# jinlong17/DA-Detect

Measured on AMD Instinct MI355X. Metric: train images/sec, DA-Faster-RCNN R-50 Cityscapes->Foggy, higher is better.
Workload: dtype f32

## Files before the change

da_detect_amd/_C.py:

```python
import contextlib
import os
import ctypes
import time

import torch

from . import _lib
from . import amax as _amax
from . import weights as _weights
from ._lib import ConvDesc

CL = torch.channels_last

NMS_TIE_RULE = 0

PROFILER = None
_KNAME_CACHE = {}


class KernelProfiler(object):

    def __init__(self, pool=0, only=None):
        self.only = only
        self._pool = []
# ... 686 lines not shown
def maxpool3x3s2_relu_backward(y, gp, scale=None):
    _dev(y, "y"), _dev(gp, "gp")
    y, gp = _nhwc(y), _nhwc(gp)
    N, C, H, W = y.shape
    Ho, Wo = (H + 2 - 3) // 2 + 1, (W + 2 - 3) // 2 + 1
    assert tuple(gp.shape) == (N, C, Ho, Wo), "maxpool3x3s2_relu_backward: gp %s for y %s" % (tuple(gp.shape), tuple(y.shape))
    g = torch.empty((N, C, H, W), dtype=torch.float32, device=y.device, memory_format=CL)
    slot = _amax.new_slot(y.device) if _mode4() else None
    _lib.call("dadet_maxpool3x3s2_relu_backward", _p(y), _p(gp), _p(scale), _p(g), N, H, W, C, Ho, Wo,
              ctypes.c_void_p(slot[0]) if slot else None, _stream())
    if slot:
        _amax.attach(g, slot)
    return g


def avgpool_forward(x):
    _dev(x, "x")
    x = _nhwc(x)
    R, C, h, w = x.shape
    y = torch.empty((R, C), dtype=torch.float32, device=x.device)
    _lib.call("dadet_avgpool_forward", _p(x), _p(y), R, h * w, C, _stream())
    return _amax.carry(y, x)


def avgpool_backward(gy, h, w):
    _dev(gy, "gy")
    gy = gy.contiguous()
    R, C = gy.shape
    gx = torch.empty((R, C, h, w), dtype=torch.float32, device=gy.device, memory_format=CL)
    _lib.call("dadet_avgpool_backward", _p(gy), _p(gx), R, h * w, C, _stream())
    return _amax.carry(gx, gy)


def nchw3_to_nhwc4(x):
    _dev(x, "x")
    x = x.contiguous()
    N, C, H, W = x.shape
    assert C == 3
    y = torch.empty((N, 4, H, W), dtype=torch.float32, device=x.device, memory_format=CL)
    _lib.call("dadet_nchw3_to_nhwc4", _p(x), _p(y), N, H, W, _stream())
    if _mode4():
        _amax.ptr(x)
        _amax.carry(y, x)
    return y


def two_image_ends(r_cst, n_src):
    return min(max(int(n_src), 0), int(r_cst)), int(r_cst)


def da_ins_tail_forward(h, w3, b3, labels, means, r_bce, r_cst, n_src):
    return da_ins_tail_forward_n(h, w3, b3, labels, means, r_bce, r_cst, two_image_ends(r_cst, n_src))


def da_ins_tail_backward(h, w3, logits, labels, means, coef, inv_keep, r_bce, r_cst, n_src):
    return da_ins_tail_backward_n(h, w3, logits, labels, means, coef, inv_keep, r_bce, r_cst, two_image_ends(r_cst, n_src))


def _row_ends(row_end):
    ends = [int(e) for e in row_end]
    return (ctypes.c_int * len(ends))(*ends), len(ends)


def da_ins_tail_forward_n(h, w3, b3, labels, means, r_bce, r_cst, row_end):
    _dev(h, "h")
    rows, C = h.shape
# ... 655 lines not shown
```

da_detect_amd/_lib.py:

```python
import ctypes
import os
from ctypes import POINTER, c_char_p, c_float, c_int, c_int64, c_size_t, c_uint64, c_void_p

_HERE = os.path.dirname(os.path.abspath(__file__))
LIB_PATH = os.environ.get("DADET_LIB") or os.path.join(_HERE, "libdadet_hip.so")
_lib = None
DEFAULT_GEMM_MODE = "4"


class ConvDesc(ctypes.Structure):

    _fields_ = [(n, c_int) for n in (
        "N", "H", "W", "Cin", "Cout", "KH", "KW", "stride", "pad", "Ho", "Wo", "OutH", "OutW",
        "out_spatial_stride", "relu_mode")]


class ConvPlanInfo(ctypes.Structure):

    _fields_ = [(n, c_int) for n in (
        "family", "variant", "tiles_m", "tiles_n", "ksplit", "splits", "rows_per_split", "sk_dp_tiles", "sk_tiles", "sk_units",
        "sk_iters", "sk_max_parts", "big_splits", "big_body", "launches", "grid", "needs_counters")] + [
        ("workspace_bytes", c_size_t), ("name", ctypes.c_char * 64)]


# ... 126 lines not shown
    "dadet_gather_pixel_taps_level": [_P, _P, _P, c_int, c_int, c_int, c_int, c_int, c_int, c_int, c_int, c_int, _P, _P],
    "dadet_scatter_pixel_taps_add_level": [_P, _P, _P, c_int, c_int, c_int, c_int, c_int, c_int, c_int, c_int, c_int, _P,
                                           _P],
    "dadet_gather_pixel_taps": [_P, _P, c_int, c_int, c_int, c_int, c_int, c_int, c_int, c_int, _P, _P],
    "dadet_scatter_pixel_taps_add": [_P, _P, c_int, c_int, c_int, c_int, c_int, c_int, c_int, c_int, _P, _P],
    "dadet_fast_rcnn_loss": [_P, _P, c_int, c_int, _P, _P, c_int, _P, _P, _P, c_int, _P, _P, _P, _P],
    "dadet_fast_rcnn_loss_rows": [_P, _P, c_int, c_int, c_int, _P, _P, _P, _P, _P, _P],
    "dadet_sample_rois": [_P, _P, _P, c_int, c_int, c_int, c_uint64, c_int, _P, _P, _P, _P, _P, _P, _P, _P],
    "dadet_proposals_sample": [_P, _P, _P, _P, c_int, _P, c_int, _P, _P, c_int, c_float, c_float, c_float, c_float, c_float,
                               c_float, c_int, c_int, c_uint64, c_int, _P, _P, _P, _P, _P, _P, _P, _P, _P, _P, _P, _P],
    "dadet_sample_anchors": [_P, _P, c_int, c_int, c_int, c_uint64, c_int64, _P, _P, _P, _P, _P],
    "dadet_topk_sorted": [_P, c_int, c_int, c_int64, c_int, _P, _P, _P],
    "dadet_topk_sorted_rows_workspace_bytes": [c_int, c_int, POINTER(c_size_t)],
    "dadet_topk_sorted_rows": [POINTER(TopkRow), c_int, _P, c_size_t, _P],
    "dadet_rpn_anchor_targets": [_P, _P, c_int, _P, c_int, c_float, c_float, _P, _P, _P, _P],
    "dadet_box_match_encode": [_P, c_int, _P, _P, c_int, c_float, c_float, c_float, c_float, c_float, c_float, _P, _P,
                               _P, _P],
    "dadet_roi_pool_forward": [_P, _P, _P, _P, c_int, c_int, c_int, c_int, c_int, c_int, c_int, c_float, _P],
    "dadet_roi_pool_backward": [_P, _P, _P, _P, c_int, c_int, c_int, c_int, c_int, c_int, c_int, _P],
    "dadet_deform_psroi_pool_forward": [_P, _P, _P, _P, _P, c_int, c_int, c_int, c_int, c_int, c_int, c_float,
                                        c_int, c_int, c_int, c_int, c_int, c_float, c_int, _P],
    "dadet_deform_psroi_pool_backward": [_P, _P, _P, _P, _P, _P, _P, c_int, c_int, c_int, c_int, c_int, c_int,
                                         c_float, c_int, c_int, c_int, c_int, c_int, c_float, c_int, _P],
    "dadet_relu_bn_backward": [_P, _P, _P, _P, _P, c_int64, c_int, _P],
    "dadet_relu_bn_backward_m": [_P, _P, _P, _P, _P, c_int64, c_int, _P, _P, _P],
    "dadet_colsum_workspace_bytes": [c_int64, c_int, POINTER(c_size_t)],
    "dadet_colsum": [_P, _P, c_int64, c_int, _P, c_size_t, _P],
    "dadet_colsum_ld": [_P, c_int, _P, c_int64, c_int, c_int, _P, c_size_t, _P],
    "dadet_channel_affine": [_P, _P, _P, _P, c_int64, c_int, c_int, _P],
    "dadet_maxpool3x3s2_forward": [_P, _P, c_int, c_int, c_int, c_int, c_int, c_int, _P],
    "dadet_maxpool3x3s2_relu_backward": [_P, _P, _P, _P, c_int, c_int, c_int, c_int, c_int, c_int, _P, _P],
    "dadet_avgpool_forward": [_P, _P, c_int, c_int, c_int, _P],
    "dadet_avgpool_backward": [_P, _P, c_int, c_int, c_int, _P],
    "dadet_nchw3_to_nhwc4": [_P, _P, c_int, c_int, c_int, _P],
    "dadet_rpn_decode_clip": [_P, _P, _P, c_int, c_float, c_float, c_float, c_float, c_float, c_float, c_float, _P, _P],
    "dadet_da_img_head_loss_forward": [_P, _P, _P, _P, _P, _P, c_int, c_int, c_int, _P],
    "dadet_da_img_head_loss_backward": [_P, _P, _P, _P, _P, _P, _P, _P, _P, c_int, c_int, c_int, _P],
    "dadet_da_img_head_loss_backward_g": [_P, _P, _P, _P, _P, _P, _P, c_float, c_float, _P, _P, _P, _P, c_int, c_int, c_int,
                                          _P],
    "dadet_da_img_head_loss_backward_gm": [_P, _P, _P, _P, _P, _P, _P, c_float, c_float, _P, _P, _P, _P, c_int, c_int, c_int,
                                          _P, _P, _P],
    "dadet_da_ins_tail_forward": [_P, _P, _P, _P, _P, _P, _P, c_int, c_int, c_int, c_int, c_int, _P],
    "dadet_da_ins_tail_backward": [_P, _P, _P, _P, _P, _P, c_float, _P, _P, _P, _P, c_int, c_int, c_int, c_int, c_int, _P],
    "dadet_da_ins_tail_forward_n": [_P, _P, _P, _P, _P, _P, _P, c_int, c_int, POINTER(c_int), c_int, c_int, c_int, _P],
    "dadet_da_ins_tail_backward_n": [_P, _P, _P, _P, _P, _P, c_float, _P, _P, _P, _P, c_int, c_int, POINTER(c_int), c_int,
                                     c_int, c_int, _P],
    "dadet_da_ins_dropout_rows": [_P, _P, _P, c_int64, c_int, _P],
    "dadet_da_ins_merge": [_P, _P, _P, _P, _P, _P, c_int64, c_int, _P],
    "dadet_triplet_w_forward": [_P, _P, _P, c_int, c_int, c_int, c_float, c_float, _P, _P, _P],
    "dadet_triplet_w_backward": [_P, _P, _P, _P, _P, c_int, c_int, c_int, c_float, c_float, _P, _P, _P, _P],
    "dadet_sgd_step": [_P, c_int, c_int64, c_float, c_int, c_float, _P],
}
_RESTYPES = {"dadet_last_error": c_char_p}
EXPORTED_SYMBOLS = sorted(list(_SIGNATURES) + ["dadet_last_error"])


class DadetError(RuntimeError):
    pass


def load():
    global _lib
    if _lib is not None:
        return _lib
    if not os.path.exists(LIB_PATH):
        raise DadetError(
# ... 27 lines not shown
```

da_detect_amd/csrc/elementwise.hip:

```cpp
#include "box_match.h"
#include "conv_common.h"
#include <float.h>

namespace dadet {

static inline int stream_blocks(int64_t work_items, int threads) {
  int64_t b = ceil_div64(work_items, threads);
  if (b > kMaxStreamBlocks) b = kMaxStreamBlocks;
  if (b < 1) b = 1;
  return (int)b;
}

__global__ void relu_bn_backward_kernel(const float4* __restrict__ g, const float4* __restrict__ y,
                                        const float4* __restrict__ scale, float4* __restrict__ g_out,
                                        float4* __restrict__ g_scaled, int64_t total4, int C4,
                                        unsigned* __restrict__ amax_out, unsigned* __restrict__ amax_scaled) {
  float mo = 0.f, ms = 0.f;
  for (int64_t i = (int64_t)blockIdx.x * blockDim.x + threadIdx.x; i < total4;
       i += (int64_t)gridDim.x * blockDim.x) {
    const float4 gv = g[i];
    float4 r = gv;
    if (y) {
      const float4 yv = y[i];
      r.x = yv.x > 0.f ? gv.x : 0.f;
// ... 158 lines not shown
}

__global__ void avgpool_fwd_kernel(const float4* __restrict__ x, float4* __restrict__ y, int R, int HW,
                                   int C4) {
  const int64_t total = (int64_t)R * C4;
  const float inv = (float)HW;
  for (int64_t i = (int64_t)blockIdx.x * blockDim.x + threadIdx.x; i < total;
       i += (int64_t)gridDim.x * blockDim.x) {
    const int c = (int)(i % C4);
    const int64_t r = i / C4;
    float4 a = make_float4(0.f, 0.f, 0.f, 0.f);
    for (int p = 0; p < HW; ++p) {
      const float4 v = x[(r * HW + p) * C4 + c];
      a.x += v.x; a.y += v.y; a.z += v.z; a.w += v.w;
    }
    a.x /= inv; a.y /= inv; a.z /= inv; a.w /= inv;
    y[i] = a;
  }
}
__global__ void avgpool_bwd_kernel(const float4* __restrict__ gy, float4* __restrict__ gx, int R, int HW,
                                   int C4) {
  const int64_t total = (int64_t)R * HW * C4;
  const float inv = (float)HW;
  for (int64_t i = (int64_t)blockIdx.x * blockDim.x + threadIdx.x; i < total;
       i += (int64_t)gridDim.x * blockDim.x) {
    const int c = (int)(i % C4);
    const int64_t r = i / ((int64_t)HW * C4);
    float4 g = gy[r * C4 + c];
    g.x /= inv; g.y /= inv; g.z /= inv; g.w /= inv;
    gx[i] = g;
  }
}

__global__ void nchw3_to_nhwc4_kernel(const float* __restrict__ x, float4* __restrict__ y, int N,
                                      int64_t HW) {
  const int64_t total = (int64_t)N * HW;
  for (int64_t i = (int64_t)blockIdx.x * blockDim.x + threadIdx.x; i < total;
       i += (int64_t)gridDim.x * blockDim.x) {
    const int64_t n = i / HW, p = i % HW;
    const float* b = x + n * 3 * HW + p;
    y[i] = make_float4(b[0], b[HW], b[2 * HW], 0.f);
  }
}

__global__ void rpn_decode_clip_kernel(const float4* __restrict__ deltas, const float4* __restrict__ anchors,
                                       const int64_t* __restrict__ topk_idx, int K, float wx, float wy,
                                       float ww, float wh, float xform_clip, float im_w, float im_h,
                                       float4* __restrict__ out) {
  const int k = blockIdx.x * blockDim.x + threadIdx.x;
  if (k >= K) return;
  const int64_t a = topk_idx[k];
  const float4 b = anchors[a];
  const float4 d = deltas[a];
  const float width = b.z - b.x + 1.f;
  const float height = b.w - b.y + 1.f;
  const float ctr_x = b.x + 0.5f * width;
  const float ctr_y = b.y + 0.5f * height;
  const float dx = d.x / wx, dy = d.y / wy;
  float dw = d.z / ww, dh = d.w / wh;
  dw = fminf(dw, xform_clip);
  dh = fminf(dh, xform_clip);
  const float pcx = dx * width + ctr_x;
  const float pcy = dy * height + ctr_y;
  const float pw = expf(dw) * width;
  const float ph = expf(dh) * height;
  float x1 = pcx - 0.5f * pw;
// ... 302 lines not shown
  DADET_REQUIRE(N >= 0 && H > 0 && W > 0 && C > 0 && C % 4 == 0, "maxpool_relu_backward: bad dims");
  DADET_REQUIRE(Ho == (H + 2 - 3) / 2 + 1 && Wo == (W + 2 - 3) / 2 + 1, "maxpool_relu_backward: Ho/Wo mismatch");
  if (N == 0) return DADET_OK;
  DADET_REQUIRE(y && gp && g && aligned16(y) && aligned16(gp) && aligned16(scale) && aligned16(g),
                "maxpool_relu_backward: bad pointers");
  DADET_REQUIRE((int64_t)N * H * W < (1LL << 31), "maxpool_relu_backward: tensor too large for 32-bit pixel indexing");
  const int64_t total = (int64_t)N * H * W * (C / 4);
  hipLaunchKernelGGL(maxpool3x3s2_relu_backward_kernel, dim3(stream_blocks(total, 256)), dim3(256), 0, as_stream(stream),
                     reinterpret_cast<const float4*>(y), reinterpret_cast<const float4*>(gp),
                     reinterpret_cast<const float4*>(scale), reinterpret_cast<float4*>(g), N, H, W, C / 4, Ho, Wo,
                     reinterpret_cast<unsigned*>(amax_out));
  return check_launch("maxpool3x3s2_relu_backward");
}

extern "C" int dadet_avgpool_forward(const float* x, float* y, int R, int HW, int C, void* stream) {
  DADET_REQUIRE(R >= 0 && HW > 0 && C > 0 && C % 4 == 0, "avgpool: bad dims");
  if (R == 0) return DADET_OK;
  DADET_REQUIRE(x && y && aligned16(x) && aligned16(y), "avgpool: bad pointers");
  hipLaunchKernelGGL(avgpool_fwd_kernel, dim3(stream_blocks((int64_t)R * (C / 4), 256)), dim3(256), 0,
                     as_stream(stream), reinterpret_cast<const float4*>(x), reinterpret_cast<float4*>(y), R,
                     HW, C / 4);
  return check_launch("avgpool_forward");
}
extern "C" int dadet_avgpool_backward(const float* gy, float* gx, int R, int HW, int C, void* stream) {
  DADET_REQUIRE(R >= 0 && HW > 0 && C > 0 && C % 4 == 0, "avgpool_backward: bad dims");
  if (R == 0) return DADET_OK;
  DADET_REQUIRE(gy && gx && aligned16(gy) && aligned16(gx), "avgpool_backward: bad pointers");
  hipLaunchKernelGGL(avgpool_bwd_kernel, dim3(stream_blocks((int64_t)R * HW * (C / 4), 256)), dim3(256), 0,
                     as_stream(stream), reinterpret_cast<const float4*>(gy), reinterpret_cast<float4*>(gx),
                     R, HW, C / 4);
  return check_launch("avgpool_backward");
}

extern "C" int dadet_nchw3_to_nhwc4(const float* x, float* y, int N, int H, int W, void* stream) {
  DADET_REQUIRE(N >= 0 && H > 0 && W > 0, "nchw3_to_nhwc4: bad dims");
  if (N == 0) return DADET_OK;
  DADET_REQUIRE(x && y && aligned16(y), "nchw3_to_nhwc4: bad pointers");
  const int64_t HW = (int64_t)H * W;
  hipLaunchKernelGGL(nchw3_to_nhwc4_kernel, dim3(stream_blocks((int64_t)N * HW, 256)), dim3(256), 0,
                     as_stream(stream), x, reinterpret_cast<float4*>(y), N, HW);
  return check_launch("nchw3_to_nhwc4");
}

extern "C" int dadet_rpn_decode_clip(const float* deltas, const float* anchors, const int64_t* topk_idx,
                                     int K, float wx, float wy, float ww, float wh, float xform_clip,
                                     float im_w, float im_h, float* boxes_out, void* stream) {
  DADET_REQUIRE(K >= 0, "rpn_decode_clip: K < 0");
  if (K == 0) return DADET_OK;
  DADET_REQUIRE(deltas && anchors && topk_idx && boxes_out, "rpn_decode_clip: null pointer");
  DADET_REQUIRE(aligned16(deltas) && aligned16(anchors) && aligned16(boxes_out),
                "rpn_decode_clip: pointers must be 16-byte aligned");
  hipLaunchKernelGGL(rpn_decode_clip_kernel, dim3(ceil_div(K, 256)), dim3(256), 0, as_stream(stream),
                     reinterpret_cast<const float4*>(deltas), reinterpret_cast<const float4*>(anchors),
                     topk_idx, K, wx, wy, ww, wh, xform_clip, im_w, im_h,
                     reinterpret_cast<float4*>(boxes_out));
  return check_launch("rpn_decode_clip");
}

extern "C" int dadet_rpn_anchor_targets(const float* anchors, const unsigned char* visible, int A,
                                        const float* gt_boxes, int G, float high_threshold, float low_threshold,
                                        unsigned* workspace_G, float* labels, float* regression_targets,
                                        void* stream) {
  DADET_REQUIRE(A >= 0 && G > 0, "rpn_anchor_targets: needs A >= 0 anchors and G > 0 ground-truth boxes");
  if (A == 0) return DADET_OK;
  DADET_REQUIRE(anchors && visible && gt_boxes && workspace_G && labels && regression_targets,
                "rpn_anchor_targets: null pointer");
// ... 71 lines not shown
```

da_detect_amd/layers/misc.py:

```python

import torch
from torch import nn
from torch.autograd import Function
from torch.autograd.function import once_differentiable

from .. import _C
from .. import amax as _amax
from .conv import conv2d_affine_act

CL = torch.channels_last


class FrozenBatchNorm2d(nn.Module):

    def __init__(self, n):
        super(FrozenBatchNorm2d, self).__init__()
        self.register_buffer("weight", torch.ones(n))
        self.register_buffer("bias", torch.zeros(n))
        self.register_buffer("running_mean", torch.zeros(n))
        self.register_buffer("running_var", torch.ones(n))
        self._cache = None

    def folded(self):
        key = (self.weight._version, self.bias._version, self.running_mean._version,
               self.running_var._version, self.weight.device)
        if self._cache is None or self._cache[0] != key:
            scale = self.weight * self.running_var.rsqrt()
            shift = self.bias - self.running_mean * scale
            self._cache = (key, scale.contiguous(), shift.contiguous())
        return self._cache[1], self._cache[2]

    def forward(self, x):
        scale, shift = self.folded()
        return _ChannelAffine.apply(x, scale, shift)


class _ChannelAffine(Function):
    @staticmethod
    def forward(ctx, x, scale, shift):
# ... 235 lines not shown
    @staticmethod
    def forward(ctx, logits, targets, gamma, alpha):
        ctx.save_for_backward(logits, targets)
        ctx.num_classes, ctx.gamma, ctx.alpha = logits.shape[1], gamma, alpha
        return _C.sigmoid_focalloss_forward(logits, targets, ctx.num_classes, gamma, alpha)

    @staticmethod
    @once_differentiable
    def backward(ctx, d_loss):
        logits, targets = ctx.saved_tensors
        return _C.sigmoid_focalloss_backward(logits, targets, d_loss.contiguous(), ctx.num_classes, ctx.gamma,
                                             ctx.alpha), None, None, None


sigmoid_focal_loss = _SigmoidFocalLoss.apply


class SigmoidFocalLoss(nn.Module):

    def __init__(self, gamma, alpha):
        super(SigmoidFocalLoss, self).__init__()
        self.gamma, self.alpha = gamma, alpha

    def forward(self, logits, targets):
        return sigmoid_focal_loss(logits, targets, self.gamma, self.alpha).sum()

    def __repr__(self):
        return "{}(gamma={}, alpha={})".format(self.__class__.__name__, self.gamma, self.alpha)


class _AvgPoolHW(Function):

    @staticmethod
    def forward(ctx, x):
        ctx.hw = (x.shape[2], x.shape[3])
        return _C.avgpool_forward(x)

    @staticmethod
    @once_differentiable
    def backward(ctx, g):
        return _C.avgpool_backward(g, *ctx.hw)


_POOL_MEMO = True


def global_avg_pool(x):
    if x.shape[0] == 0:
        return x.new_empty((0, x.shape[1]))
    memo = x.__dict__.get("_dadet_pooled") if _POOL_MEMO else None
    if memo is not None and memo[0] == x._version and memo[1] == torch.is_grad_enabled():
        return memo[2]
    y = _AvgPoolHW.apply(x)
    x._dadet_pooled = (x._version, torch.is_grad_enabled(), y)
    return y
```

da_detect_amd/modeling/backbone/resnet.py:

```python
import weakref
from collections import namedtuple

import torch
import torch.nn.functional as F
from torch import nn

from ... import _C
from ...layers import Conv2d, FrozenBatchNorm2d, conv2d_affine_act
from ...utils.registry import Registry
from ...utils import streams
from ...utils.streams import WgradLane
from ...weights import Stamp

StageSpec = namedtuple("StageSpec", ["index", "block_count", "return_features"])


def _specs(*rows):
    return tuple(StageSpec(index=i, block_count=c, return_features=r) for (i, c, r) in rows)


ResNet50StagesTo5 = _specs((1, 3, False), (2, 4, False), (3, 6, False), (4, 3, True))
ResNet50StagesTo4 = _specs((1, 3, False), (2, 4, False), (3, 6, True))
ResNet101StagesTo5 = _specs((1, 3, False), (2, 4, False), (3, 23, False), (4, 3, True))
ResNet101StagesTo4 = _specs((1, 3, False), (2, 4, False), (3, 23, True))
ResNet50FPNStagesTo5 = _specs((1, 3, True), (2, 4, True), (3, 6, True), (4, 3, True))
ResNet101FPNStagesTo5 = _specs((1, 3, True), (2, 4, True), (3, 23, True), (4, 3, True))
ResNet152FPNStagesTo5 = _specs((1, 3, True), (2, 8, True), (3, 36, True), (4, 3, True))


_WGRAD_BATCH = True
_WGRAD_GROUP = __import__("os").environ.get("DADET_WGRAD_GROUP", "1") == "1"


class _WgradGroup(object):

    _known = {}

    def __init__(self, lane, batch, weights):
        self.lane, self.batch, self.reqs = lane, batch, []
        self.on = (_WGRAD_GROUP and batch is not None and _C._mode4() and 2 <= len(weights) <= _C.WGRAD_GROUP_MAX
# ... 6 lines not shown
    def take(self, w, xin, gout, stride, pad, scale, shape=None):
        if not self.on:
            return False
        self.reqs.append(dict(x=xin, gy=gout, weight_shape=tuple(w.shape) if shape is None else shape, stride=stride,
                              pad=pad, out_scale=scale, dw=streams.direct_grad_target(w), accumulate=True))
        return True

    def issue(self):
        if not self.reqs:
            return
        reqs, batch = self.reqs, self.batch
        key = self.key + tuple((tuple(r["x"].shape), r["stride"]) for r in reqs)

        def run():
            ok = self._known.get(key, True) and _C.conv_wgrad_group(reqs, batch)
            if not ok:
                self._known[key] = self._known[self.key] = False
                for r in reqs:
                    _C.conv_wgrad(r["x"], r["gy"], r["weight_shape"], r["stride"], r["pad"], out_scale=r["out_scale"],
                                  dw=r["dw"], accumulate=True, pending=batch)

        self.lane.run_group(run, *[t for r in reqs for t in (r["x"], r["gy"])])
        self.reqs = []


class _BlockBackward(object):

    def __init__(self, needs, x, w1, wd, s1, sd, stride):
        self.need_x, self.n1, self.n2, self.n3, nd = needs
        self.nd = nd and wd is not None
        self.x, self.w1, self.wd, self.s1, self.sd, self.stride = x, w1, wd, s1, sd, stride

    def open(self, G, out, out_private, y2, w2, w3, s3):
        self.S3 = G.contiguous(memory_format=torch.channels_last) if out_private else _C.relu_bn_backward(G, out, None)[1]
        self.lane = WgradLane(G.device, rows=G.shape[0] * G.shape[2] * G.shape[3])
        self.batch = _C.WgradBatch() if _WGRAD_BATCH else None
        weights = ((w3, self.n3), (w2, self.n2), (self.w1, self.n1), (self.wd, self.nd))
        self.group = _WgradGroup(self.lane, self.batch, [w for w, need in weights if need])
        dw3 = self.wgrad(w3, y2, self.S3, 1, 0, s3) if self.n3 else None
        return _C.conv_forward(self.S3, _C.conv_weight_transpose(w3, s3), relu_mode=2, mask_ref=y2), dw3

    def wgrad(self, w, xin, gout, st, pd, sc, shape=None, grouped=True):
        shape = tuple(w.shape) if shape is None else shape
        batch = self.batch
        if grouped and self.group.take(w, xin, gout, st, pd, sc, shape=shape):
            return None
        return self.lane.run_into(w, lambda acc: _C.conv_wgrad(xin, gout, shape, st, pd, out_scale=sc, dw=acc,
                                                               accumulate=True, pending=batch),
                                  lambda: _C.conv_wgrad(xin, gout, shape, st, pd, out_scale=sc, pending=batch),
                                  xin, gout)

    def close(self, S1, in_relu):
        x, w1, wd, s1, sd, stride, S3 = self.x, self.w1, self.wd, self.s1, self.sd, self.stride, self.S3
        dw1 = dwd = dx = None
        if self.n1:
            dw1 = self.wgrad(w1, x, S1, stride, 0, s1)
        if self.nd:
            dwd = self.wgrad(wd, x, S3, stride, 0, sd)
        self.group.issue()
        self.lane.reduce_batch(self.batch)
        if self.need_x:
            gate = dict(relu_mode=2, mask_ref=x) if in_relu else {}
            hw = tuple(x.shape[2:])
            if wd is None:
                dx = _C.conv_forward(S1, _C.conv_weight_transpose(w1, s1), addend=S3, **gate)
            elif stride == 1:
                t = _C.conv_forward(S3, _C.conv_weight_transpose(wd, sd))
# ... 148 lines not shown
        self.downsample = None
        if in_channels != out_channels:
            self.downsample = nn.Sequential(
                Conv2d(in_channels, out_channels, kernel_size=1, stride=stride, bias=False),
                norm_func(out_channels))
            nn.init.kaiming_uniform_(self.downsample[0].weight, a=1)
        stride_1x1, stride_3x3 = (stride, 1) if stride_in_1x1 else (1, stride)
        self.conv1 = Conv2d(in_channels, bottleneck_channels, kernel_size=1, stride=stride_1x1, bias=False)
        self.bn1 = norm_func(bottleneck_channels)
        self.with_dcn = bool(dcn_config.get("stage_with_dcn", False))
        if self.with_dcn:
            from ...layers.dcn import DFConv2d
            self.conv2 = DFConv2d(bottleneck_channels, bottleneck_channels,
                                  with_modulated_dcn=dcn_config.get("with_modulated_dcn", False), kernel_size=3,
                                  stride=stride_3x3, groups=num_groups, dilation=dilation,
                                  deformable_groups=dcn_config.get("deformable_groups", 1), bias=False)
        else:
            self.conv2 = Conv2d(bottleneck_channels, bottleneck_channels, kernel_size=3, stride=stride_3x3,
                                padding=1, bias=False)
        self.bn2 = norm_func(bottleneck_channels)
        self.conv3 = Conv2d(bottleneck_channels, out_channels, kernel_size=1, bias=False)
        self.bn3 = norm_func(out_channels)
        for l in (self.conv1, self.conv3) + (() if self.with_dcn else (self.conv2,)):
            nn.init.kaiming_uniform_(l.weight, a=1)

    def forward(self, x, in_relu=False, out_private=False, stride=None):
        if self.with_dcn:
            assert stride is None
            if self._dcn_fusable(x):
                c2 = self.conv2
                wd = sd = bd = None
                if self.downsample is not None:
                    wd, (sd, bd) = self.downsample[0].weight, self.downsample[1].folded()
                return _DCNBottleneckFn.apply(x, self.conv1.weight, c2.conv.weight, self.conv3.weight, wd,
                                              c2.offset.weight, c2.offset.bias, *self.bn1.folded(), *self.bn2.folded(),
                                              *self.bn3.folded(), sd, bd, self.conv1.stride[0], in_relu, out_private,
                                              c2.with_modulated_dcn, c2.conv.deformable_groups)
            return self._forward_dcn(x)
        if self.conv2.stride[0] == 1:
            if x.shape[0] == 0 and stride is None:
                return self._forward_per_conv(x)
            wd = sd = bd = None
            if self.downsample is not None:
                wd, (sd, bd) = self.downsample[0].weight, self.downsample[1].folded()
            return _BottleneckFn.apply(x, self.conv1.weight, self.conv2.weight, self.conv3.weight, wd,
                                       *self.bn1.folded(), *self.bn2.folded(), *self.bn3.folded(), sd, bd,
                                       self.conv1.stride[0] if stride is None else stride, in_relu, out_private)
        assert stride is None
        return self._forward_per_conv(x)

    def input_is_strided_1x1(self):
        s = self.conv1.stride[0]
        if (self.uses_fused_path() and s > 1 and self.downsample is not None and self.conv1.kernel_size == (1, 1)
                and self.downsample[0].kernel_size == (1, 1) and self.downsample[0].stride[0] == s):
            return s
        return 1

    def uses_fused_path(self):
        if self.with_dcn:
            return self._dcn_fusable(None)
        return self.conv2.stride[0] == 1

    def _dcn_fusable(self, x):
        c = self.conv2.conv
        ok = (_DCN_FUSED and c.stride == 1 and c.dilation == 1 and c.groups == 1 and c.bias is None
              and c.kernel_size == (3, 3) and c.in_channels % (4 * c.deformable_groups) == 0)
        return ok and (x is None or (x.is_cuda and x.shape[0] > 0))

    def _forward_dcn(self, x):
        out = self.conv1(x, *self.bn1.folded(), relu=True)
        out = F.relu(self.bn2(self.conv2(out)))
        identity = x if self.downsample is None else self.downsample[0](x, *self.downsample[1].folded())
        return self.conv3(out, *self.bn3.folded(), residual=identity, relu=True)

    def _forward_per_conv(self, x):
        out = self.conv1(x, *self.bn1.folded(), relu=True)
        out = self.conv2(out, *self.bn2.folded(), relu=True)
        identity = x if self.downsample is None else self.downsample[0](x, *self.downsample[1].folded())
        return self.conv3(out, *self.bn3.folded(), residual=identity, relu=True)

# ... 180 lines not shown
```

da_detect_amd/modeling/rpn/rpn.py:

```python
import os

import torch
from torch import nn

from ...layers import Conv2d, conv1x1_multi
from ...layers.misc import rpn_head_loss_rows, rpn_head_loss_rows_pyramid
from .. import registry
from ..box_coder import BoxCoder
from .anchor_generator import make_anchor_generator
from .inference import make_rpn_postprocessor
from .loss import make_rpn_loss_evaluator
from ..elision import elision_enabled, leading_source_images
from ...utils.streams import record, side_section, side_stream



@registry.RPN_HEADS.register("SingleConvRPNHead")
class RPNHead(nn.Module):

    def __init__(self, cfg, in_channels, num_anchors):
        super(RPNHead, self).__init__()
        self.conv = Conv2d(in_channels, in_channels, kernel_size=3, stride=1, padding=1)
        self.cls_logits = Conv2d(in_channels, num_anchors, kernel_size=1, stride=1)
        self.bbox_pred = Conv2d(in_channels, num_anchors * 4, kernel_size=1, stride=1)
        for l in (self.conv, self.cls_logits, self.bbox_pred):
            torch.nn.init.normal_(l.weight, std=0.01)
            torch.nn.init.constant_(l.bias, 0)

    keep_hidden = False

    def forward(self, x):
        logits, bbox_reg = [], []
        self.hidden = []
        for feature in x:
            t = self.conv(feature, relu=True)
            if self.keep_hidden:
                self.hidden.append(t)
            cls, box = conv1x1_multi(t, [self.cls_logits.weight, self.bbox_pred.weight],
                                     [self.cls_logits.bias, self.bbox_pred.bias])
            logits.append(cls)
            bbox_reg.append(box)
        return logits, bbox_reg


_ROW_BACKWARD = __import__("os").environ.get("DADET_RPN_ROW_BACKWARD", "1") == "1"


class _InjectGrad(torch.autograd.Function):

    @staticmethod
    def forward(ctx, x, g, e, event):
        ctx.event = event
        ctx.save_for_backward(*[t for t in (g, e) if t is not None])
        ctx.has = (g is not None, e is not None)
        from ... import amax
        return amax.carry(x.view_as(x), x)

    @staticmethod
    def backward(ctx, grad_out):
        saved = list(ctx.saved_tensors)
        g = saved.pop(0) if ctx.has[0] else None
        e = saved.pop(0) if ctx.has[1] else None
        if ctx.event is not None:
            torch.cuda.current_stream(grad_out.device).wait_event(ctx.event)
        out = grad_out + e if e is not None else None
        if g is not None:
            if out is None and g.shape[0] == grad_out.shape[0]:
                out = grad_out + g
            else:
                out = grad_out.clone() if out is None else out
                out[:g.shape[0]] += g
        return out, None, None, None


class RPNModule(torch.nn.Module):

    early_backward = False
    live_images = None
    after_early_backward = None

    def __init__(self, cfg):
        super(RPNModule, self).__init__()
        self.cfg = cfg.clone()
        anchor_generator = make_anchor_generator(cfg)
        in_channels = cfg.MODEL.BACKBONE.OUT_CHANNELS
        head = registry.RPN_HEADS[cfg.MODEL.RPN.RPN_HEAD](cfg, in_channels,
                                                         anchor_generator.num_anchors_per_location()[0])
        rpn_box_coder = BoxCoder(weights=(1.0, 1.0, 1.0, 1.0))
        self.anchor_generator = anchor_generator
        self.head = head
        self.box_selector_train = make_rpn_postprocessor(cfg, rpn_box_coder, is_train=True)
        self.box_selector_test = make_rpn_postprocessor(cfg, rpn_box_coder, is_train=False)
        self.loss_evaluator = make_rpn_loss_evaluator(cfg, rpn_box_coder)
        self.proposals_ready = None
        self._feature_grads = None
        self.inputs_ready = None

# ... 143 lines not shown
```

include/dadet.h:

```cpp
#ifndef DADET_H_
#define DADET_H_

#include <stddef.h>
#include <stdint.h>

#ifdef __cplusplus
extern "C" {
#endif

#define DADET_OK 0
#define DADET_EINVAL (-1)
#define DADET_ELAUNCH (-2)
#define DADET_EWORKSPACE (-3)
#define DADET_EUNSUPPORTED (-4)

const char* dadet_last_error(void);
int dadet_version(void);
int dadet_device_info(int* cu_count, int* clock_khz, size_t* hbm_bytes, char* arch_name, int arch_name_len);

int dadet_nms_workspace_bytes(int n, size_t* bytes_out);
int dadet_nms(const float* boxes_xyxy, const float* scores, int n, float thresh, int tie_rule,
              int max_keep, void* workspace, size_t workspace_bytes, int64_t* keep_out,
              int* num_keep_out, void* stream);
int dadet_nms_batch_workspace_bytes(int batch, int n_max, size_t* bytes_out);
// ... 296 lines not shown

int dadet_box_match_encode(const float* proposals, int P, const float* gt_boxes, const int64_t* gt_labels, int G,
                           float high_threshold, float low_threshold, float wx, float wy, float ww, float wh,
                           int64_t* matched_idxs, int64_t* labels, float* regression_targets, void* stream);

int dadet_deform_psroi_pool_forward(const float* data, const float* rois, const float* trans, float* out,
                                    float* top_count, int B, int H, int W, int C, int R, int no_trans,
                                    float spatial_scale, int output_dim, int group_size, int pooled_size,
                                    int part_size, int sample_per_part, float trans_std, int num_classes,
                                    void* stream);
int dadet_deform_psroi_pool_backward(const float* grad_out, const float* top_count, const float* data,
                                     const float* rois, const float* trans, float* grad_data, float* grad_trans,
                                     int B, int H, int W, int C, int R, int no_trans, float spatial_scale,
                                     int output_dim, int group_size, int pooled_size, int part_size,
                                     int sample_per_part, float trans_std, int num_classes, void* stream);

int dadet_relu_bn_backward(const float* g, const float* y, const float* scale, float* g_out,
                           float* g_scaled, int64_t rows, int C, void* stream);
int dadet_relu_bn_backward_m(const float* g, const float* y, const float* scale, float* g_out, float* g_scaled,
                             int64_t rows, int C, float* amax_out, float* amax_scaled, void* stream);
int dadet_colsum_workspace_bytes(int64_t rows, int C, size_t* bytes_out);
int dadet_colsum_ld(const float* g, int ld, float* out, int64_t rows, int C, int accumulate, void* workspace,
                    size_t workspace_bytes, void* stream);
int dadet_colsum(const float* g, float* out, int64_t rows, int C, void* workspace, size_t workspace_bytes,
                 void* stream);
int dadet_channel_affine(const float* x, const float* scale, const float* bias, float* y, int64_t rows,
                         int C, int relu, void* stream);
int dadet_maxpool3x3s2_forward(const float* x, float* y, int N, int H, int W, int C, int Ho, int Wo,
                               void* stream);
int dadet_maxpool3x3s2_relu_backward(const float* y, const float* gp, const float* scale, float* g, int N, int H,
                                     int W, int C, int Ho, int Wo, float* amax_out, void* stream);
int dadet_avgpool_forward(const float* x, float* y, int R, int HW, int C, void* stream);
int dadet_avgpool_backward(const float* gy, float* gx, int R, int HW, int C, void* stream);
int dadet_nchw3_to_nhwc4(const float* x, float* y, int N, int H, int W, void* stream);

int dadet_rpn_decode_clip(const float* deltas, const float* anchors, const int64_t* topk_idx, int K,
                          float wx, float wy, float ww, float wh, float xform_clip, float im_w,
                          float im_h, float* boxes_out, void* stream);

int dadet_da_img_head_loss_forward(const float* t, const float* w2, const float* b2, const float* labels,
                                   float* logits_out, float* sums_out, int num_images,
                                   int rows_per_image, int C1, void* stream);
int dadet_da_img_head_loss_backward(const float* t, const float* w2, const float* logits,
                                    const float* labels, const float* coef, float* g_t_w, float* g_t_x,
                                    float* g_w2, float* g_b2, int num_images, int rows_per_image, int C1,
                                    void* stream);
int dadet_da_img_head_loss_backward_g(const float* t, const float* w2, const float* logits, const float* labels,
                                      const float* g_bce, const float* g_mean_sig, const float* w_adv_dev, float w_adv,
                                      float w_cst, float* g_t_w, float* g_t_x, float* g_w2, float* g_b2, int num_images,
                                      int rows_per_image, int C1, void* stream);
int dadet_da_img_head_loss_backward_gm(const float* t, const float* w2, const float* logits, const float* labels,
                                       const float* g_bce, const float* g_mean_sig, const float* w_adv_dev, float w_adv,
                                       float w_cst, float* g_t_w, float* g_t_x, float* g_w2, float* g_b2, int num_images,
                                       int rows_per_image, int C1, float* amax_w, float* amax_x, void* stream);
int dadet_da_ins_tail_forward(const float* h, const float* w3, const float* b3, const float* labels,
                              const float* means, float* logits, float* sums, int R_bce, int R_cst, int n_src,
                              int levels, int C, void* stream);
int dadet_da_ins_tail_backward(const float* h, const float* w3, const float* logits, const float* labels,
                               const float* means, const float* coef, float inv_keep, float* g_z, float* g_w3,
                               float* g_b3, float* g_means, int R_bce, int R_cst, int n_src, int levels, int C,
                               void* stream);
int dadet_da_ins_tail_forward_n(const float* h, const float* w3, const float* b3, const float* labels,
                                const float* means, float* logits, float* sums, int R_bce, int R_cst,
                                const int* row_end, int num_images, int levels, int C, void* stream);
int dadet_da_ins_tail_backward_n(const float* h, const float* w3, const float* logits, const float* labels,
                                 const float* means, const float* coef, float inv_keep, float* g_z, float* g_w3,
// ... 26 lines not shown
```

Before: 170.8.

## Fuse ReLU gating into gradient junction and lazy avgpool backward

Adds two fused kernels. One sums the incoming gradient with the side-branch gradients and applies the ReLU mask of the backbone output in a single pass. The other expands the avgpool gradient and applies the ReLU mask directly. Tensors are tagged so the bottleneck backward can skip its own relu_bn_backward pass when the gradient is already gated, or materialise the pooled gradient lazily. This removes full-size elementwise passes and intermediate tensors over large feature maps, at the cost of version-tagged metadata that must stay correct across autograd.

```diff
diff --git a/da_detect_amd/_C.py b/da_detect_amd/_C.py
--- a/da_detect_amd/_C.py
+++ b/da_detect_amd/_C.py
@@ -742,6 +742,39 @@
     return _amax.carry(gx, gy)
 
 
+def avgpool_backward_gated(gy, y):
+    _dev(gy, "gy"), _dev(y, "y")
+    gy = gy.contiguous()
+    y = _nhwc(y)
+    R, C, h, w = y.shape
+    assert tuple(gy.shape) == (R, C)
+    gx = torch.empty((R, C, h, w), dtype=torch.float32, device=gy.device, memory_format=CL)
+    slot = _amax.new_slot(gy.device) if _mode4() and R > 0 else None
+    _lib.call("dadet_avgpool_backward_gated", _p(gy), _p(y), _p(gx), ctypes.c_void_p(slot[0]) if slot else None, R, h * w, C,
+              _stream())
+    if slot:
+        _amax.attach(gx, slot)
+    return gx
+
+
+def grad_junction(grad, y, e=None, g=None):
+    _dev(grad, "grad"), _dev(y, "y")
+    grad, y = _nhwc(grad), _nhwc(y)
+    assert grad.shape == y.shape
+    B, C, H, W = y.shape
+    e = _nhwc(e) if e is not None else None
+    g = _nhwc(g) if g is not None else None
+    assert e is None or e.shape == y.shape
+    assert g is None or (tuple(g.shape[1:]) == (C, H, W) and g.shape[0] <= B)
+    out = torch.empty_like(grad)
+    slot = _amax.new_slot(y.device) if _mode4() and grad.numel() > 0 else None
+    _lib.call("dadet_grad_junction", _p(grad), _p(e), _p(g), 0 if g is None else g.shape[0] * H * W, _p(y), _p(out),
+              ctypes.c_void_p(slot[0]) if slot else None, B * H * W, C, _stream())
+    if slot:
+        _amax.attach(out, slot)
+    return out
+
+
 def nchw3_to_nhwc4(x):
     _dev(x, "x")
     x = x.contiguous()
diff --git a/da_detect_amd/_lib.py b/da_detect_amd/_lib.py
--- a/da_detect_amd/_lib.py
+++ b/da_detect_amd/_lib.py
@@ -182,6 +182,8 @@
     "dadet_maxpool3x3s2_relu_backward": [_P, _P, _P, _P, c_int, c_int, c_int, c_int, c_int, c_int, _P, _P],
     "dadet_avgpool_forward": [_P, _P, c_int, c_int, c_int, _P],
     "dadet_avgpool_backward": [_P, _P, c_int, c_int, c_int, _P],
+    "dadet_avgpool_backward_gated": [_P, _P, _P, _P, c_int, c_int, c_int, _P],
+    "dadet_grad_junction": [_P, _P, _P, c_int64, _P, _P, _P, c_int64, c_int, _P],
     "dadet_nchw3_to_nhwc4": [_P, _P, c_int, c_int, c_int, _P],
     "dadet_rpn_decode_clip": [_P, _P, _P, c_int, c_float, c_float, c_float, c_float, c_float, c_float, c_float, _P, _P],
     "dadet_da_img_head_loss_forward": [_P, _P, _P, _P, _P, _P, c_int, c_int, c_int, _P],
diff --git a/da_detect_amd/csrc/elementwise.hip b/da_detect_amd/csrc/elementwise.hip
--- a/da_detect_amd/csrc/elementwise.hip
+++ b/da_detect_amd/csrc/elementwise.hip
@@ -214,6 +214,51 @@
   }
 }
 
+__global__ void avgpool_bwd_gated_kernel(const float4* __restrict__ gy, const float4* __restrict__ y,
+                                         float4* __restrict__ gx, int R, int HW, int C4, unsigned* __restrict__ amax) {
+  const int64_t total = (int64_t)R * HW * C4;
+  const float inv = (float)HW;
+  float mo = 0.f;
+  for (int64_t i = (int64_t)blockIdx.x * blockDim.x + threadIdx.x; i < total;
+       i += (int64_t)gridDim.x * blockDim.x) {
+    const int c = (int)(i % C4);
+    const int64_t r = i / ((int64_t)HW * C4);
+    float4 g = gy[r * C4 + c];
+    g.x /= inv; g.y /= inv; g.z /= inv; g.w /= inv;
+    const float4 yv = y[i];
+    float4 o;
+    o.x = yv.x > 0.f ? g.x : 0.f; o.y = yv.y > 0.f ? g.y : 0.f;
+    o.z = yv.z > 0.f ? g.z : 0.f; o.w = yv.w > 0.f ? g.w : 0.f;
+    gx[i] = o;
+    mo = fmaxf(fmaxf(mo, fmaxf(fabsf(o.x), fabsf(o.y))), fmaxf(fabsf(o.z), fabsf(o.w)));
+  }
+  if (amax) amax_publish(amax, mo);
+}
+
+__global__ void grad_junction_kernel(const float4* __restrict__ grad, const float4* __restrict__ e,
+                                     const float4* __restrict__ g, int64_t total4_g, const float4* __restrict__ y,
+                                     float4* __restrict__ out, int64_t total4, unsigned* __restrict__ amax) {
+  float mo = 0.f;
+  for (int64_t i = (int64_t)blockIdx.x * blockDim.x + threadIdx.x; i < total4;
+       i += (int64_t)gridDim.x * blockDim.x) {
+    float4 v = grad[i];
+    if (e) {
+      const float4 a = e[i];
+      v.x = v.x + a.x; v.y = v.y + a.y; v.z = v.z + a.z; v.w = v.w + a.w;
+    }
+    if (i < total4_g) {
+      const float4 a = g[i];
+      v.x = v.x + a.x; v.y = v.y + a.y; v.z = v.z + a.z; v.w = v.w + a.w;
+    }
+    const float4 yv = y[i];
+    v.x = yv.x > 0.f ? v.x : 0.f; v.y = yv.y > 0.f ? v.y : 0.f;
+    v.z = yv.z > 0.f ? v.z : 0.f; v.w = yv.w > 0.f ? v.w : 0.f;
+    out[i] = v;
+    mo = fmaxf(fmaxf(mo, fmaxf(fabsf(v.x), fabsf(v.y))), fmaxf(fabsf(v.z), fabsf(v.w)));
+  }
+  if (amax) amax_publish(amax, mo);
+}
+
 __global__ void nchw3_to_nhwc4_kernel(const float* __restrict__ x, float4* __restrict__ y, int N,
                                       int64_t HW) {
   const int64_t total = (int64_t)N * HW;
@@ -582,6 +627,34 @@
   return check_launch("avgpool_backward");
 }
 
+extern "C" int dadet_avgpool_backward_gated(const float* gy, const float* y, float* gx, float* amax, int R, int HW, int C,
+                                            void* stream) {
+  DADET_REQUIRE(R >= 0 && HW > 0 && C > 0 && C % 4 == 0, "avgpool_backward_gated: bad dims");
+  if (R == 0) return DADET_OK;
+  DADET_REQUIRE(gy && y && gx && aligned16(gy) && aligned16(y) && aligned16(gx), "avgpool_backward_gated: bad pointers");
+  hipLaunchKernelGGL(avgpool_bwd_gated_kernel, dim3(stream_blocks((int64_t)R * HW * (C / 4), 256)), dim3(256), 0,
+                     as_stream(stream), reinterpret_cast<const float4*>(gy), reinterpret_cast<const float4*>(y),
+                     reinterpret_cast<float4*>(gx), R, HW, C / 4, reinterpret_cast<unsigned*>(amax));
+  return check_launch("avgpool_backward_gated");
+}
+
+extern "C" int dadet_grad_junction(const float* grad, const float* e, const float* g, int64_t rows_g, const float* y,
+                                   float* out, float* amax, int64_t rows, int C, void* stream) {
+  DADET_REQUIRE(rows >= 0 && C > 0 && C % 4 == 0, "grad_junction: C=%d must be a multiple of 4", C);
+  DADET_REQUIRE(rows_g >= 0 && rows_g <= rows && (g || rows_g == 0), "grad_junction: rows_g=%lld of %lld", (long long)rows_g,
+                (long long)rows);
+  if (rows == 0) return DADET_OK;
+  DADET_REQUIRE(grad && y && out, "grad_junction: null pointer");
+  DADET_REQUIRE(aligned16(grad) && aligned16(e) && aligned16(g) && aligned16(y) && aligned16(out),
+                "grad_junction: pointers must be 16-byte aligned");
+  const int64_t total4 = rows * (C / 4);
+  hipLaunchKernelGGL(grad_junction_kernel, dim3(stream_blocks(total4, 256)), dim3(256), 0, as_stream(stream),
+                     reinterpret_cast<const float4*>(grad), reinterpret_cast<const float4*>(e),
+                     reinterpret_cast<const float4*>(g), rows_g * (C / 4), reinterpret_cast<const float4*>(y),
+                     reinterpret_cast<float4*>(out), total4, reinterpret_cast<unsigned*>(amax));
+  return check_launch("grad_junction");
+}
+
 extern "C" int dadet_nchw3_to_nhwc4(const float* x, float* y, int N, int H, int W, void* stream) {
   DADET_REQUIRE(N >= 0 && H > 0 && W > 0, "nchw3_to_nhwc4: bad dims");
   if (N == 0) return DADET_OK;
diff --git a/da_detect_amd/gates.py b/da_detect_amd/gates.py
--- /dev/null
+++ b/da_detect_amd/gates.py
@@ -0,0 +1,40 @@
+import os
+
+
+def enabled():
+    return os.environ.get("DADET_GRAD_JUNCTIONS", "1")[:1] != "0"
+
+
+def mark_relu(t):
+    t._dadet_relu = t._version
+    return t
+
+
+def is_relu(t):
+    return t.__dict__.get("_dadet_relu") == t._version
+
+
+def _key(y):
+    return (y.data_ptr(), tuple(y.shape), tuple(y.stride()))
+
+
+def mark_gated(grad, y):
+    grad._dadet_gated = (_key(y), grad._version)
+    return grad
+
+
+def gated_for(grad, y):
+    return grad.__dict__.get("_dadet_gated") == (_key(y), grad._version)
+
+
+def mark_unpooled(grad, gy):
+    grad._dadet_unpooled = (gy, grad._version, gy._version)
+    return grad
+
+
+def unpooled_source(grad):
+    a = grad.__dict__.get("_dadet_unpooled")
+    if (a is None or a[1] != grad._version or a[2] != a[0]._version or grad.dim() != 4
+            or tuple(a[0].shape) != tuple(grad.shape[:2]) or tuple(grad.stride()[2:]) != (0, 0)):
+        return None
+    return a[0]
diff --git a/da_detect_amd/layers/misc.py b/da_detect_amd/layers/misc.py
--- a/da_detect_amd/layers/misc.py
+++ b/da_detect_amd/layers/misc.py
@@ -5,6 +5,7 @@
 from torch.autograd.function import once_differentiable
 
 from .. import _C
+from .. import gates
 from .. import amax as _amax
 from .conv import conv2d_affine_act
 
@@ -306,14 +307,19 @@
 class _AvgPoolHW(Function):
 
     @staticmethod
-    def forward(ctx, x):
+    def forward(ctx, x, lazy):
         ctx.hw = (x.shape[2], x.shape[3])
+        ctx.lazy = lazy
         return _C.avgpool_forward(x)
 
     @staticmethod
     @once_differentiable
     def backward(ctx, g):
-        return _C.avgpool_backward(g, *ctx.hw)
+        h, w = ctx.hw
+        if ctx.lazy and g.shape[0] > 0:
+            g = g.contiguous()
+            return gates.mark_unpooled((g / float(h * w))[:, :, None, None].expand(-1, -1, h, w), g), None
+        return _C.avgpool_backward(g, h, w), None
 
 
 _POOL_MEMO = True
@@ -325,6 +331,6 @@
     memo = x.__dict__.get("_dadet_pooled") if _POOL_MEMO else None
     if memo is not None and memo[0] == x._version and memo[1] == torch.is_grad_enabled():
         return memo[2]
-    y = _AvgPoolHW.apply(x)
+    y = _AvgPoolHW.apply(x, x.is_cuda and x.shape[1] % 4 == 0 and gates.is_relu(x) and gates.enabled())
     x._dadet_pooled = (x._version, torch.is_grad_enabled(), y)
     return y
diff --git a/da_detect_amd/modeling/backbone/resnet.py b/da_detect_amd/modeling/backbone/resnet.py
--- a/da_detect_amd/modeling/backbone/resnet.py
+++ b/da_detect_amd/modeling/backbone/resnet.py
@@ -6,6 +6,7 @@
 from torch import nn
 
 from ... import _C
+from ... import gates
 from ...layers import Conv2d, FrozenBatchNorm2d, conv2d_affine_act
 from ...utils.registry import Registry
 from ...utils import streams
@@ -78,7 +79,12 @@
         self.x, self.w1, self.wd, self.s1, self.sd, self.stride = x, w1, wd, s1, sd, stride
 
     def open(self, G, out, out_private, y2, w2, w3, s3):
-        self.S3 = G.contiguous(memory_format=torch.channels_last) if out_private else _C.relu_bn_backward(G, out, None)[1]
+        gated = out_private or gates.gated_for(G, out)
+        pooled = None if gated else gates.unpooled_source(G)
+        if pooled is not None:
+            self.S3 = _C.avgpool_backward_gated(pooled, out)
+        else:
+            self.S3 = G.contiguous(memory_format=torch.channels_last) if gated else _C.relu_bn_backward(G, out, None)[1]
         self.lane = WgradLane(G.device, rows=G.shape[0] * G.shape[2] * G.shape[3])
         self.batch = _C.WgradBatch() if _WGRAD_BATCH else None
         weights = ((w3, self.n3), (w2, self.n2), (self.w1, self.n1), (self.wd, self.nd))
@@ -293,10 +299,10 @@
                 wd = sd = bd = None
                 if self.downsample is not None:
                     wd, (sd, bd) = self.downsample[0].weight, self.downsample[1].folded()
-                return _DCNBottleneckFn.apply(x, self.conv1.weight, c2.conv.weight, self.conv3.weight, wd,
-                                              c2.offset.weight, c2.offset.bias, *self.bn1.folded(), *self.bn2.folded(),
-                                              *self.bn3.folded(), sd, bd, self.conv1.stride[0], in_relu, out_private,
-                                              c2.with_modulated_dcn, c2.conv.deformable_groups)
+                return gates.mark_relu(_DCNBottleneckFn.apply(
+                    x, self.conv1.weight, c2.conv.weight, self.conv3.weight, wd, c2.offset.weight, c2.offset.bias,
+                    *self.bn1.folded(), *self.bn2.folded(), *self.bn3.folded(), sd, bd, self.conv1.stride[0], in_relu,
+                    out_private, c2.with_modulated_dcn, c2.conv.deformable_groups))
             return self._forward_dcn(x)
         if self.conv2.stride[0] == 1:
             if x.shape[0] == 0 and stride is None:
@@ -304,9 +310,9 @@
             wd = sd = bd = None
             if self.downsample is not None:
                 wd, (sd, bd) = self.downsample[0].weight, self.downsample[1].folded()
-            return _BottleneckFn.apply(x, self.conv1.weight, self.conv2.weight, self.conv3.weight, wd,
-                                       *self.bn1.folded(), *self.bn2.folded(), *self.bn3.folded(), sd, bd,
-                                       self.conv1.stride[0] if stride is None else stride, in_relu, out_private)
+            return gates.mark_relu(_BottleneckFn.apply(
+                x, self.conv1.weight, self.conv2.weight, self.conv3.weight, wd, *self.bn1.folded(), *self.bn2.folded(),
+                *self.bn3.folded(), sd, bd, self.conv1.stride[0] if stride is None else stride, in_relu, out_private))
         assert stride is None
         return self._forward_per_conv(x)
 
diff --git a/da_detect_amd/modeling/rpn/rpn.py b/da_detect_amd/modeling/rpn/rpn.py
--- a/da_detect_amd/modeling/rpn/rpn.py
+++ b/da_detect_amd/modeling/rpn/rpn.py
@@ -11,6 +11,7 @@
 from .inference import make_rpn_postprocessor
 from .loss import make_rpn_loss_evaluator
 from ..elision import elision_enabled, leading_source_images
+from ... import gates
 from ...utils.streams import record, side_section, side_stream
 
 
@@ -51,8 +52,9 @@
     @staticmethod
     def forward(ctx, x, g, e, event):
         ctx.event = event
-        ctx.save_for_backward(*[t for t in (g, e) if t is not None])
-        ctx.has = (g is not None, e is not None)
+        fuse = x.is_cuda and x.dim() == 4 and x.shape[1] % 4 == 0 and gates.is_relu(x) and gates.enabled()
+        ctx.save_for_backward(*[t for t in (g, e, x if fuse else None) if t is not None])
+        ctx.has = (g is not None, e is not None, fuse)
         from ... import amax
         return amax.carry(x.view_as(x), x)
 
@@ -61,8 +63,12 @@
         saved = list(ctx.saved_tensors)
         g = saved.pop(0) if ctx.has[0] else None
         e = saved.pop(0) if ctx.has[1] else None
+        y = saved.pop(0) if ctx.has[2] else None
         if ctx.event is not None:
             torch.cuda.current_stream(grad_out.device).wait_event(ctx.event)
+        if y is not None and grad_out.dtype == torch.float32:
+            from ... import _C
+            return gates.mark_gated(_C.grad_junction(grad_out, y, e, g), y), None, None, None
         out = grad_out + e if e is not None else None
         if g is not None:
             if out is None and g.shape[0] == grad_out.shape[0]:
diff --git a/include/dadet.h b/include/dadet.h
--- a/include/dadet.h
+++ b/include/dadet.h
@@ -352,6 +352,10 @@
                                      int W, int C, int Ho, int Wo, float* amax_out, void* stream);
 int dadet_avgpool_forward(const float* x, float* y, int R, int HW, int C, void* stream);
 int dadet_avgpool_backward(const float* gy, float* gx, int R, int HW, int C, void* stream);
+int dadet_avgpool_backward_gated(const float* gy, const float* y, float* gx, float* amax, int R, int HW, int C,
+                                 void* stream);
+int dadet_grad_junction(const float* grad, const float* e, const float* g, int64_t rows_g, const float* y, float* out,
+                        float* amax, int64_t rows, int C, void* stream);
 int dadet_nchw3_to_nhwc4(const float* x, float* y, int N, int H, int W, void* stream);
 
 int dadet_rpn_decode_clip(const float* deltas, const float* anchors, const int64_t* topk_idx, int K,
```

Result: no change. 171.6, median of 6 (+0.5%).
